# hanishkvc/prgs-sdr-kspecanal

Measured on AMD Instinct MI355X. Metric: windowed FFTs/sec, fftSize=4096, 50% overlap, hanning (zeroSpan hot path incl. Max/Min/Avg/Cur + waterfall), higher is better.
Workload: dtype f32

## Files before the change

prgs-sdr-kspecanal_amd/build.py:

```python
import os
import shutil
import subprocess
import sys

HERE = os.path.dirname(os.path.abspath(__file__))
SRC = os.path.join(HERE, "csrc", "ksa_api.hip")
OUT = os.path.join(HERE, "libksa.so")
FLAGS = ["--offload-arch=gfx950", "-O3", "-std=c++17", "-fno-slp-vectorize", "-Wno-unused-value",
         "-shared", "-fPIC"]


def sources():
    d = os.path.join(HERE, "csrc")
    return [os.path.join(d, f) for f in sorted(os.listdir(d))] + [os.path.join(HERE, "..", "include", "ksa.h")]


def is_stale():
    if not os.path.exists(OUT):
        return True
    t = os.path.getmtime(OUT)
    return any(os.path.getmtime(s) > t for s in sources())


def build(force=False, verbose=False):
    if not force and not is_stale():
        return OUT
    hipcc = shutil.which("hipcc") or "/opt/rocm/bin/hipcc"
    cmd = [hipcc] + FLAGS + ["-o", OUT + ".tmp", SRC]
    if verbose:
        print(" ".join(cmd))
    r = subprocess.run(cmd, capture_output=True, text=True)
    if r.returncode != 0:
        raise RuntimeError("hipcc failed:\n" + r.stdout + r.stderr)
    os.replace(OUT + ".tmp", OUT)
    return OUT


if __name__ == "__main__":
    print(build(force="--force" in sys.argv, verbose=True))
```

prgs-sdr-kspecanal_amd/csrc/ksa_api.hip:

```cpp
#include <hip/hip_runtime.h>

#include <algorithm>
#include <climits>
#include <cmath>
#include <cstdarg>
#include <cstdio>
#include <cstdlib>
#include <cstring>
#include <mutex>
#include <string>
#include <type_traits>
#include <vector>

#include "../../include/ksa.h"
#include "ksa_dif16.hpp"
#include "ksa_kernels.hpp"
#include "ksa_kernels32.hpp"
#include "ksa_kernels64.hpp"
#include "ksa_kernels_pair.hpp"
#include "ksa_kernels_mr.hpp"
#include "ksa_pfb.hpp"
#include "ksa_tables.hpp"

namespace {
// ... 55 lines not shown
  hipStream_t stream = nullptr;
  int num_cu = 0;
  int* d_starts = nullptr;
  int* d_start_last = nullptr;
  float* d_window = nullptr;
  float* d_window32 = nullptr;
  float2* d_tw_mid = nullptr;
  float2* d_tw_last = nullptr;
  float* d_adj = nullptr;
  float* d_scan_adj = nullptr;
  void* d_iq_stage = nullptr;
  float* d_frames = nullptr;
  float* d_part = nullptr;
  float* d_xchg = nullptr;
  float* d_partial = nullptr;
  float* d_state = nullptr;
  float* d_hm = nullptr;
  float* d_scan_state = nullptr;
  float* d_scan_hm = nullptr;
  float* d_scan_avg_rows = nullptr;
  float* d_levels = nullptr;
  int* d_highs = nullptr;
  float* d_parts = nullptr;
  int levels_cap = 0;
  float* d_gather = nullptr;
  size_t gather_cap = 0;
  void* d_scan_stage = nullptr;
  size_t scan_stage_cap = 0;
  float* d_scan_rows = nullptr;
  int scan_rows = 0;
  int scan_rows_passes = 0;
  float* d_scan_halo = nullptr;
  float* d_scan_send = nullptr;
  size_t scan_halo_cap = 0, scan_send_cap = 0;
  hipEvent_t ev_ready = nullptr, ev_copied = nullptr, ev_stream = nullptr;
  hipStream_t copy_stream = nullptr;
  void* d_slot[2] = {nullptr, nullptr};
  size_t slot_cap[2] = {0, 0};
  hipEvent_t ev_slot_copied[2] = {nullptr, nullptr}, ev_slot_read[2] = {nullptr, nullptr}, ev_copy_start = nullptr;
  float* d_host_rows = nullptr;
  size_t host_rows_cap = 0;
  int plan_frames = 0;
  int sub_n = 0;
  float2* d_dif_tw = nullptr;
  float2* d_dif_z = nullptr;
  float* d_dif_y = nullptr;
// ... 93 lines not shown
    return f(int_c<ksa::CUMU_AVG>{});
  }
  if (p.cumu == ksa::CUMU_AVG) return f(int_c<ksa::CUMU_AVG>{});
  if (p.cumu == ksa::CUMU_MAX) return f(int_c<ksa::CUMU_MAX>{});
  return f(int_c<ksa::CUMU_MIN>{});
}
constexpr bool fold_avg_or_psd(int cm) { return cm == ksa::CUMU_AVG || cm == ksa::CUMU_PSD; }

struct KernelFit {
  int vgprs = 0, blocks_per_cu = 1;
};
template <class K>
int configure_kernel(K kfn, int threads, int lds_bytes, KernelFit* fit, int lds_attr = -1) {
  HIP_OK(hipFuncSetAttribute(reinterpret_cast<const void*>(kfn), hipFuncAttributeMaxDynamicSharedMemorySize, lds_attr < 0 ? lds_bytes : lds_attr));
  hipFuncAttributes attr;
  HIP_OK(hipFuncGetAttributes(&attr, reinterpret_cast<const void*>(kfn)));
  int occ = 0;
  HIP_OK(hipOccupancyMaxActiveBlocksPerMultiprocessor(&occ, kfn, threads, lds_bytes));
  fit->vgprs = attr.numRegs;
  fit->blocks_per_cu = std::max(1, occ);
  return 0;
}

template <class K>
int launch_split(ksa_engine* e, K kfn, const SpecParams& p, int n, int threads, int lds_bytes, bool may_split, int grid_cap) {
  const int capacity = e->num_cu * e->blocks_per_cu;
  SpecParams q = p;
  const int plan = plan_of(e, p);
  if (e->d_parts && may_split && !exp_env("KSA_NO_SPLIT") && p.nwin > 1 && plan * 2 <= capacity) {
    q.parts = std::min(p.nwin, capacity / plan);
    q.part_out = e->d_parts;
  }
  int grid = std::max(1, std::min(q.nframes * std::max(1, q.parts), capacity));
  grid = std::max(1, std::min(grid, grid_cap));
  hipLaunchKernelGGL(kfn, dim3(grid), dim3(threads), lds_bytes, e->stream, q);
  if (q.parts > 1) {
    hipLaunchKernelGGL(ksa::combine_parts_kernel, dim3((n / 4 + 63) / 64, q.nframes), dim3(64), 0, e->stream, q, n);
    if (q.hm_w > 0)
      hipLaunchKernelGGL(ksa::rowmax_batch, dim3((q.hm_w + 255) / 256, q.nframes), dim3(256), 0, e->stream, q, n);
  }
  HIP_OK(hipGetLastError());
  return 0;
}

template <int N, int FMT, int RM, int CM>
int launch_pair_c(ksa_engine* e, const SpecParams& p, bool configure_only) {
  using PP = ksa::PlanPair<N>;
  auto kfn = ksa::spectrum_pair_kernel<N, FMT, RM, CM>;
  if (configure_only) {
    KernelFit fit;
    if (configure_kernel(kfn, ksa::Plan<N>::T, PP::LDS_BYTES, &fit)) return 1;
    if (FMT == ksa::FMT_C64 && fold_avg_or_psd(CM)) {
      e->pair_bpc = fit.blocks_per_cu;
      e->pair_vgprs = fit.vgprs;
      e->pair_lds = PP::LDS_BYTES;
    }
    return 0;
  }
  const int npairs = (p.nframes + 1) / 2;
  const int grid = std::max(1, std::min(npairs, e->num_cu * e->pair_bpc));
  hipLaunchKernelGGL(kfn, dim3(grid), dim3(ksa::Plan<N>::T), PP::LDS_BYTES, e->stream, p);
  HIP_OK(hipGetLastError());
  return 0;
}

template <int N, int FMT, int RM>
int launch_pair(ksa_engine* e, const SpecParams& p, bool cfg_only) {
  return with_fold(e, p, cfg_only, [&](auto cm) { return launch_pair_c<N, FMT, RM, decltype(cm)::value>(e, p, cfg_only); });
}

template <int N, int FMT, int RM, int CM>
int launch_spec_c(ksa_engine* e, const SpecParams& p, bool configure_only) {
  using P = ksa::Plan<N>;
  auto kfn = ksa::spectrum_kernel<N, FMT, RM, CM>;
  static const int lds_pad = exp_env("KSA_LDS_PAD_KB") ? atoi(exp_env("KSA_LDS_PAD_KB")) * 1024 : 0;
  const int lds_bytes = ksa::Tune<N>::LDS_BYTES + lds_pad;
  if (configure_only) {
    KernelFit fit;
    if (configure_kernel(kfn, P::T, lds_bytes, &fit)) return 1;
    if (FMT == ksa::FMT_C64) {
      e->threads = P::T;
      e->lds_bytes = ksa::Tune<N>::LDS_BYTES;
      e->vgprs = fit.vgprs;
      e->blocks_per_cu = fit.blocks_per_cu;
    }
    return 0;
  }
  return launch_split(e, kfn, p, N, P::T, lds_bytes, N >= 1024, INT_MAX);
}

template <int N, int FMT, int RM>
int launch_spec_t(ksa_engine* e, const SpecParams& p, bool configure_only) {
#ifdef KSA_EXPERIMENTS
  constexpr bool pair_size = ksa::Plan<N>::S == 1 && ksa::Plan<N>::T <= 256 && ksa::Plan<N>::M >= 2;
#else
  constexpr bool pair_size = N == 1024;
#endif
  if constexpr (pair_size) {
    if (e->pair_ok) {
      if (configure_only) {
        if (RM != 0 && launch_pair<N, FMT, 0>(e, p, true)) return 1;
        if (RM != 4 && launch_pair<N, FMT, 4>(e, p, true)) return 1;
        if (RM != 8 && launch_pair<N, FMT, 8>(e, p, true)) return 1;
        if (launch_pair<N, FMT, RM>(e, p, true)) return 1;
      } else if (plan_of(e, p) >= 2 * e->num_cu * e->pair_bpc) return launch_pair<N, FMT, RM>(e, p, false);
    }
  }
  if constexpr (ksa::Tune<N>::fold_const(RM)) {
    return with_fold(e, p, configure_only, [&](auto cm) { return launch_spec_c<N, FMT, RM, decltype(cm)::value>(e, p, configure_only); });
  } else {
    if (fold_psd(e)) return launch_spec_c<N, FMT, RM, ksa::CUMU_PSD>(e, p, configure_only);
// ... 26 lines not shown
    return 0;
  }
  const char* g = exp_env("KSA_GRID");
  return launch_split(e, kfn, p, N, P::T, P::LDS_BYTES, true, g ? atoi(g) : INT_MAX);
}

template <int N, int FMT>
int launch_spec32(ksa_engine* e, const SpecParams& p, bool cfg_only) {
  return with_fold(e, p, cfg_only, [&](auto cm) { return launch_spec32_c<N, FMT, decltype(cm)::value>(e, p, cfg_only); });
}

template <int CM, bool W1>
int launch_spec64_c(ksa_engine* e, const SpecParams& p, bool configure_only) {
  auto kfn = ksa::spectrum64_kernel<ksa::FMT_C64, CM, W1>;
  if (configure_only) {
    KernelFit fit;
    if (configure_kernel(kfn, ksa::Plan64::T, ksa::Plan64::LDS_BYTES, &fit)) return 1;
    if (fold_avg_or_psd(CM)) {
      e->k64_bpc = fit.blocks_per_cu;
      e->k64_vgprs = fit.vgprs;
    }
    return 0;
  }
  const int grid = std::max(1, std::min(p.nframes, e->num_cu * e->k64_bpc));
  hipLaunchKernelGGL(kfn, dim3(grid), dim3(ksa::Plan64::T), ksa::Plan64::LDS_BYTES, e->stream, p);
  HIP_OK(hipGetLastError());
  return 0;
}

int launch_spec64(ksa_engine* e, const SpecParams& p, bool cfg_only) {
  const bool w1 = e->win_ones && !exp_env("KSA_NO_W1");
  return with_fold(e, p, cfg_only, [&](auto cm) {
    constexpr int CM = decltype(cm)::value;
    return w1 ? launch_spec64_c<CM, true>(e, p, cfg_only) : launch_spec64_c<CM, false>(e, p, cfg_only);
  });
}

template <int FMT>
int launch_spec_n(ksa_engine* e, const SpecParams& p, bool cfg_only) {
  const int rm = p.nwin > 1 ? e->reuse_m : 0;
  if (e->plan32) return e->sub_n == 8192 ? launch_spec32<8192, FMT>(e, p, cfg_only) : launch_spec32<16384, FMT>(e, p, cfg_only);
  return with_size(e->sub_n, [&](auto size) {
    constexpr int N = decltype(size)::value;
    if constexpr (N == 64 && FMT == ksa::FMT_C64) {
      if (e->k64_ok) {
        if (cfg_only) { if (launch_spec64(e, p, true)) return 1; }
        else if (!exp_env("KSA_NO_K64")) return launch_spec64(e, p, false);
      }
// ... 151 lines not shown
          return dispatch(R, Radices{}, [&](auto radix) {
            constexpr int RX = decltype(radix)::value;
            if constexpr (RX == 16)
              hipLaunchKernelGGL(ksa::dif16_kernel<FMT>, dim3(n1 / 512, nwin, cf), dim3(256), 0, e->stream, a);
            else
              hipLaunchKernelGGL((ksa::dif_wide_kernel<FMT, RX>), dim3(n1 / 256, nwin, cf), dim3(256), 0, e->stream, a);
            return 0;
          });
        })) return 1;
    SpecParams b{};
    b.iq = e->d_dif_z;
    b.frame_stride = (long long)nwin * n1;
    b.frame_len = nwin * n1;
    b.nframes = cf * R;
    b.nwin = nwin;
    b.starts = e->d_starts_b;
    b.window = e->d_ones;
    b.tw_mid = p.tw_mid;
    b.tw_last = p.tw_last;
    b.scale = p.scale;
    b.cumu = p.cumu;
    b.out_mode = ksa::OUT_LINEAR;
    b.out = e->d_dif_y;
    e->plan_frames = chunk_frames * R;
    if (launch_spec_n<ksa::FMT_C64>(e, b, false)) return 1;
    ksa::DifFinishParams c{};
    c.y = e->d_dif_y;
    c.n = n;
    c.n1 = n1;
    c.radix = R;
    c.frame0 = f0;
    c.out_mode = p.out_mode;
    c.gain = p.gain;
    c.min_amp = p.min_amp;
    c.out = p.out;
    c.hm_w = p.hm_w;
    c.adj = p.adj;
    c.hm_rows = p.hm_rows;
    c.hm_ring = p.hm_ring;
    c.hm_index0 = p.hm_index0;
    c.hm_first = p.hm_first;
    dispatch(R, Radices{}, [&](auto radix) {
      hipLaunchKernelGGL(ksa::dif16_finish_kernel<decltype(radix)::value>, dim3(n1 / (1024 / R), cf), dim3(256), 0, e->stream, c);
      return 0;
    });
  }
// ... 28 lines not shown
  p.starts = raw ? e->d_start_last : e->d_starts;
#if defined(KSA32_TAPS_X4) && !KSA32_TAPS_X4
  p.window = e->d_window;
#else
  p.window = (e->plan32 && e->path == 0) ? e->d_window32 : e->d_window;
#endif
  p.tw_mid = e->d_tw_mid;
  p.tw_last = e->d_tw_last;
  p.scale = (float)c.mag_scale;
  p.cumu = (raw || fold || c.cumu_mode == KSA_CUMU_AVG || c.cumu_mode == KSA_CUMU_PSD) ? ksa::CUMU_AVG : c.cumu_mode == KSA_CUMU_MAX ? ksa::CUMU_MAX : ksa::CUMU_MIN;
  p.out_mode = out_mode;
  p.gain = c.gain;
  p.min_amp = c.min_amp;
  p.u8_offset = c.u8_offset;
  p.u8_inv_scale = 1.0f / c.u8_scale;
  p.out = out;
  p.hm_w = with_hm ? c.hm_width : 0;
  p.adj = with_hm ? e->d_adj : nullptr;
  p.hm_rows = with_hm ? hm_rows : nullptr;
  p.hm_ring = with_hm ? e->d_hm : nullptr;
  p.hm_index0 = (e->hm_index + f.batch_first) % KSA_HM_ROWS;
  p.hm_first = std::max(0, f.batch_frames - KSA_HM_ROWS - f.batch_first);
  e->plan_frames = f.batch_frames;
#ifdef KSA_STAMPS
  static unsigned long long* dbg = nullptr;
  const size_t dbg_n = 4096 * 16 * 12;
  if (!dbg) hipMalloc(reinterpret_cast<void**>(&dbg), dbg_n * 8);
  hipMemsetAsync(dbg, 0, dbg_n * 8, e->stream);
  p.dbg = dbg;
#endif
  ksa::u64x2* const clk = (e->prof && e->d_clk) ? reinterpret_cast<ksa::u64x2*>(e->d_clk) + (size_t)(e->clk_launches++ % ksa::CLK_SLOTS) * 2 * ksa::CLK_KEYS : nullptr;
  if (clk) hipLaunchKernelGGL(ksa::clock_stamp_kernel, dim3(ksa::CLK_WGS), dim3(64), 0, e->stream, clk, 0);
  hipEvent_t ea, eb;
  if (prof_begin(e, &ea, &eb)) return 1;
  if (fold && launch_pfb(e, *fold)) return 1;
  int rc;
  if (e->path == 2) rc = run_dif16(e, p, f.fmt, f.batch_first, f.batch_frames);
  else if (e->path == 6) rc = with_fmt(f.fmt, [&](auto fmt) { return launch_mr<decltype(fmt)::value>(e, p, false); });
  else rc = with_fmt(f.fmt, [&](auto fmt) { return launch_spec_n<decltype(fmt)::value>(e, p, false); });
  e->plan_frames = 0;
  if (rc) return rc;
#ifdef KSA_STAMPS
  if (const char* path = exp_env("KSA_STAMPS_FILE")) {
    hipStreamSynchronize(e->stream);
    std::vector<unsigned long long> h(dbg_n);
    hipMemcpy(h.data(), dbg, dbg_n * 8, hipMemcpyDeviceToHost);
    double sum[12] = {0};
    long long waves = 0;
    for (size_t w = 0; w < dbg_n / 12; ++w) {
      if (!h[w * 12 + 0] && !h[w * 12 + 7]) continue;
      ++waves;
      for (int i = 0; i < 12; ++i) sum[i] += (double)h[w * 12 + i];
    }
    if (FILE* fp = fopen(path, "a")) {
      fprintf(fp, "waves %lld nframes %d nwin %d :", waves, f.nframes, p.nwin);
      for (int i = 0; i < 12; ++i) fprintf(fp, " %.0f", waves ? sum[i] / waves : 0.0);
      fprintf(fp, "\n");
      fclose(fp);
    }
  }
#endif
  if (prof_end(e, ea, eb)) return 1;
  if (clk) hipLaunchKernelGGL(ksa::clock_stamp_kernel, dim3(ksa::CLK_WGS), dim3(64), 0, e->stream, clk, 1);
  return 0;
}

int run_spectrum(ksa_engine* e, Frames f, int out_mode, float* out, bool with_hm, float* hm_rows) {
  if (f.batch_frames < 1) f.batch_frames = f.nframes;
  if (!fold_time(e)) return run_transform(e, f, out_mode, out, with_hm, hm_rows, nullptr);
  const ksa_config& c = e->cfg;
  if (check_frames(e, f, out, hm_rows)) return 1;
  const size_t n = (size_t)c.fft_size;
  for (int f0 = 0; f0 < f.nframes; f0 += e->pfb_chunk) {
    const int nf = std::min(e->pfb_chunk, f.nframes - f0);
    const Frames fold{static_cast<const unsigned char*>(f.iq) + (size_t)f0 * (size_t)f.stride * sample_bytes(f.fmt), f.fmt, f.stride, nf};
    const Frames folded{e->d_pfb_y, KSA_FMT_C64, (long long)e->pfb_sub * c.fft_size, nf, f.batch_first + f0, f.batch_frames};
    if (run_transform(e, folded, out_mode, out + (size_t)f0 * n, with_hm, hm_rows ? hm_rows + (size_t)f0 * c.hm_width : nullptr, &fold)) return 1;
  }
  return 0;
}

int run_accumulate(ksa_engine* e, const float* db, int nframes, long long first_index, long long total) {
  const int n = e->cfg.fft_size;
  ksa::AccParams a{};
  a.db = db;
  a.n = n;
// ... 219 lines not shown
    if (const char* mb = exp_env("KSA_FS_SCRATCH_MB")) {
      const long v = atol(mb);
      if (v >= 1 && v <= (256l << 10)) budget = (size_t)v << 20;
    }
    e->dif_chunk = (int)std::min<size_t>(std::max<size_t>(1, budget / per_frame), (size_t)c.max_frames);
    e->dif_chunk = std::min(e->dif_chunk, 4095);
    if ((he = hipMalloc(reinterpret_cast<void**>(&e->d_dif_z), per_frame * e->dif_chunk)) != hipSuccess)
      return fail("hipMalloc(%zu) for the first-stage scratch: %s", per_frame * e->dif_chunk, hipGetErrorString(he));
    if ((he = hipMalloc(reinterpret_cast<void**>(&e->d_dif_y), (size_t)e->dif_chunk * n * 4)) != hipSuccess)
      return fail("hipMalloc for the second-stage output: %s", hipGetErrorString(he));
  }
  e->max_chunks = (int)std::max<size_t>(1, std::min<size_t>(128, (64u << 20) / (3 * nn * 4)));
#define ALLOC(ptr, bytes)                                                        \
  if ((he = hipMalloc(reinterpret_cast<void**>(&(ptr)), (bytes))) != hipSuccess) \
    return fail("hipMalloc(%zu) for %s: %s", (size_t)(bytes), #ptr, hipGetErrorString(he));
  ALLOC(e->d_iq_stage, (size_t)c.full_size * 8);
  ALLOC(e->d_frames, (size_t)c.max_frames * nn * 4);
  ALLOC(e->d_part, (size_t)e->max_chunks * 3 * nn * 4);
  ALLOC(e->d_xchg, (4 * nn + (size_t)KSA_HM_ROWS * c.hm_width) * 4);
  e->d_partial = e->d_xchg;
  if (c.hm_width) e->d_hm = e->d_xchg + 4 * nn;
  ALLOC(e->d_state, 4 * nn * 4);
  if (e->path != 6) ALLOC(e->d_parts, (size_t)e->num_cu * e->blocks_per_cu * (size_t)e->sub_n * 4);
  if (c.scan_total_entries) {
    ALLOC(e->d_scan_state, (size_t)4 * c.scan_total_entries * 4);
    ALLOC(e->d_scan_hm, (size_t)KSA_HM_ROWS * c.scan_hm_width * 4);
  }
#undef ALLOC
  return 0;
}

}

extern "C" {

int ksa_abi_version(void) { return KSA_ABI_VERSION; }
const char* ksa_last_error(void) { return g_err.c_str(); }

int ksa_create(const ksa_config* cfg, ksa_engine** out) {
  if (!cfg || !out) return fail("null argument");
  *out = nullptr;
  if (validate_config(cfg)) return 1;
  int ndev = 0;
  HIP_OK(hipGetDeviceCount(&ndev));
  if (cfg->device < 0 || cfg->device >= ndev) return fail("device %d not present (%d visible)", cfg->device, ndev);
  DeviceGuard dev_guard;
// ... 18 lines not shown
  if (upload_tables(e, cfg, w)) return bail(1);
  if (configure_kernels(e, w.num_windows)) return bail(1);
  if (alloc_scratch(e, w.num_windows)) return bail(1);
  if (ksa_reset_state(e)) return bail(1);
  if (cfg->scan_total_entries && scan_reset(e)) return bail(1);
  if (hipStreamSynchronize(e->stream) != hipSuccess) return bail(fail("initial sync failed"));
  *out = e;
  return 0;
}

void ksa_destroy(ksa_engine* e) {
  if (!e) return;
  DeviceGuard dev_guard;
  hipSetDevice(e->cfg.device);
  hipDeviceSynchronize();
  for (auto& pr : e->prof_events) { hipEventDestroy(pr.first); hipEventDestroy(pr.second); }
  for (hipEvent_t ev : {e->ev_ready, e->ev_copied, e->ev_stream, e->ev_copy_start, e->ev_slot_copied[0], e->ev_slot_copied[1],
                        e->ev_slot_read[0], e->ev_slot_read[1]})
    if (ev) hipEventDestroy(ev);
  if (e->copy_stream) hipStreamDestroy(e->copy_stream);
  void* ptrs[] = {e->d_slot[0], e->d_slot[1], e->d_host_rows, e->d_clk, e->d_gather, e->d_scan_stage, e->d_scan_rows, e->d_scan_halo, e->d_scan_send,
                  e->d_starts, e->d_start_last, e->d_window, e->d_window32, e->d_tw_mid, e->d_tw_last, e->d_adj, e->d_scan_adj,
                  e->d_iq_stage, e->d_frames, e->d_part, e->d_xchg, e->d_state, e->d_scan_state, e->d_scan_hm,
                  e->d_levels, e->d_parts, e->d_highs, e->d_scan_avg_rows, e->d_dif_tw, e->d_dif_z, e->d_dif_y, e->d_ones, e->d_starts_b,
                  e->d_pfb_starts, e->d_pfb_taps, e->d_pfb_y};
  for (void* p : ptrs) if (p) hipFree(p);
  delete e;
}

int ksa_set_stream(ksa_engine* e, void* hip_stream) {
  if (!e) return fail("null engine");
  hipStream_t ns = reinterpret_cast<hipStream_t>(hip_stream);
  if (ns == e->stream) return 0;
  DeviceGuard dev_guard;
  HIP_OK(hipSetDevice(e->cfg.device));
  if (!e->ev_stream) HIP_OK(hipEventCreateWithFlags(&e->ev_stream, hipEventDisableTiming));
  HIP_OK(hipEventRecord(e->ev_stream, e->stream));
  HIP_OK(hipStreamWaitEvent(ns, e->ev_stream, 0));
  e->stream = ns;
  return 0;
}

int ksa_synchronize(ksa_engine* e) {
  if (!e) return fail("null engine");
  DeviceGuard dev_guard;
  HIP_OK(hipSetDevice(e->cfg.device));
  HIP_OK(hipStreamSynchronize(e->stream));
// ... 864 lines not shown
```

prgs-sdr-kspecanal_amd/csrc/ksa_kernels.hpp:

```cpp
#pragma once
#include <hip/hip_runtime.h>
#include <stdint.h>
#include <type_traits>
#include "ksa_fft.hpp"

namespace ksa {

enum { CUMU_AVG = 1, CUMU_MAX = 2, CUMU_MIN = 3 };
enum { CUMU_PSD = 4 };
enum { OUT_LINEAR = 0, OUT_DB = 1, OUT_DB_CLIP = 2 };
enum { FMT_C64 = 0, FMT_U8 = 1, FMT_S8 = 2, FMT_S16 = 3 };
constexpr int HM_ROWS = 128;

struct SpecParams {
  const void* iq;
  long long frame_stride;
  int frame_len;
  int nframes;
  int nwin;
  const int* starts;
  const float* window;
  const float2* tw_mid;
  const float2* tw_last;
  float scale;
  int cumu;
  int out_mode;
  float gain, min_amp;
  float u8_offset, u8_inv_scale;
  float* out;
  int hm_w;
  const float* adj;
  float* hm_rows;
  float* hm_ring;
  int hm_index0;
  int hm_first;
  int parts;
  float* part_out;
  unsigned long long* dbg;
};

constexpr int CLK_WGS = 2048;
constexpr int CLK_KEYS = 4096;
constexpr int CLK_SLOTS = 16;
typedef unsigned long long u64x2 __attribute__((ext_vector_type(2)));
__global__ __launch_bounds__(64) void clock_stamp_kernel(u64x2* out, int which) {
  unsigned long long c, r;
  asm volatile("s_memtime %0\n\ts_memrealtime %1\n\ts_waitcnt lgkmcnt(0)" : "=s"(c), "=s"(r)::"memory");
  const unsigned xcc = __builtin_amdgcn_s_getreg(20 | (0 << 6) | ((4 - 1) << 11));
  const unsigned hw = __builtin_amdgcn_s_getreg(4 | (8 << 6) | ((8 - 1) << 11));
  if (threadIdx.x == 0) {
    u64x2 v;
    v.x = c;
    v.y = r;
    out[(size_t)which * CLK_KEYS + (((xcc & 15u) << 8) | (hw & 255u))] = v;
  }
}

__device__ __forceinline__ float db_of(float lin, float gain) { return fmaf(__builtin_amdgcn_logf(lin), 3.01029995663981195f, -gain); }

__device__ __forceinline__ float nan_max(float a, float b) { return __builtin_isunordered(a, b) ? __builtin_nanf("") : fmaxf(a, b); }
__device__ __forceinline__ float nan_min(float a, float b) { return __builtin_isunordered(a, b) ? __builtin_nanf("") : fminf(a, b); }
// ... 203 lines not shown
template <> struct RawOf<FMT_S8> { typedef unsigned int type; };
template <int FMT>
__device__ __forceinline__ float tap_scale(const SpecParams& p) { return FMT == FMT_U8 ? p.u8_inv_scale : fmt_fixed_scale(FMT); }
template <int FMT>
__device__ __forceinline__ float2 unpack_signed(unsigned b) {
  static_assert(FMT == FMT_S8 || FMT == FMT_S16, "signed fixed-point formats only");
  if constexpr (FMT == FMT_S8) return make_float2((float)(int)(signed char)(b & 0xff), (float)(int)(signed char)((b >> 8) & 0xff));
  else return make_float2((float)(int)(short)(b & 0xffff), (float)((int)b >> 16));
}

#ifdef KSA_STAMPS
#define KSA_STAMP(i)                                                                        \
  do {                                                                                      \
    __builtin_amdgcn_sched_barrier(0);                                                      \
    unsigned long long _t;                                                                  \
    asm volatile("s_memtime %0\n\ts_waitcnt lgkmcnt(0)" : "=s"(_t)::"memory");              \
    __builtin_amdgcn_sched_barrier(0);                                                      \
    seg[i] += _t - t_last;                                                                  \
    t_last = _t;                                                                            \
  } while (0)
#else
#define KSA_STAMP(i) do {} while (0)
#endif

#ifdef KSA_ABL_NOLDS
#define KSA_SYNC() do {} while (0)
#define KSA_LDS_ST(dst, val) do {} while (0)
#define KSA_LDS_LD(dst, src) do {} while (0)
#else
#ifdef KSA_LDS_BARRIER
#define KSA_SYNC() asm volatile("s_waitcnt lgkmcnt(0)\n\ts_barrier" ::: "memory")
#else
#define KSA_SYNC() __syncthreads()
#endif
#define KSA_LDS_ST(dst, val) (dst) = (val)
#ifndef KSA_LDS_ATOMIC_LD
#define KSA_LDS_ATOMIC_LD 1
#endif
__device__ __forceinline__ float2 lds_ld64(const float2* p) {
#if KSA_LDS_ATOMIC_LD
  const unsigned long long v = __atomic_load_n(reinterpret_cast<const unsigned long long*>(p), __ATOMIC_RELAXED);
  return make_float2(__uint_as_float((unsigned)v), __uint_as_float((unsigned)(v >> 32)));
#else
  return *p;
#endif
}
// ... 138 lines not shown
      else if constexpr (FMT == FMT_S16) raw[(q + ROT) & 15] = __builtin_amdgcn_raw_buffer_load_b32(rsrc, voff, L * q * SB, 0);
      else raw[(q + ROT) & 15] = __builtin_amdgcn_raw_buffer_load_b16(rsrc, voff, L * q * SB, 0);
#endif
    }
  };
  auto shift_raw = [&]() {
#pragma unroll
    for (int q = 0; q + RM < 16; ++q) raw[q] = raw[q + RM];
  };

#ifdef KSA_STAMPS
  unsigned long long seg[12] = {0, 0, 0, 0, 0, 0, 0, 0, 0, 0, 0, 0};
  unsigned long long t_last;
  asm volatile("s_memtime %0\n\ts_waitcnt lgkmcnt(0)" : "=s"(t_last)::"memory");
#endif
#ifndef KSA_PF
#define KSA_PF 1
#endif
  constexpr bool PF = KSA_PF && RM > 0 && N >= 2048;
#ifndef KSA_PP
#define KSA_PP 1
#endif
  constexpr bool PP = KSA_PP && PF && RM == 8 && N == 4096;
  for (int vf = blockIdx.x; vf < p.nframes * NP; vf += gridDim.x) {
    const int frame = vf / NP, part = vf - frame * NP;
    const int k_lo = (int)((long long)p.nwin * part / NP), k_hi = (int)((long long)p.nwin * (part + 1) / NP);
    const int rounds = (k_hi - k_lo + S - 1) / S;
    float acc[16];
    const float init = p.cumu == CUMU_MIN ? __builtin_inff() : 0.0f;
#pragma unroll
    for (int i = 0; i < 16; ++i) acc[i] = init;

    if constexpr (PP) {
      for (int rd0 = 0; rd0 < rounds; rd0 += 2) {
        {
          const int rd = rd0;
          constexpr int PAR = 0;
#include "ksa_window_body.inc"
        }
        if (rd0 + 1 < rounds) {
          const int rd = rd0 + 1;
          constexpr int PAR = 1;
#include "ksa_window_body.inc"
        }
      }
    } else {
      for (int rd = 0; rd < rounds; ++rd) {
        constexpr int PAR = 0;
#include "ksa_window_body.inc"
      }
    }

    float* const red = reinterpret_cast<float*>(lds);
    __syncthreads();
    KSA_STAMP(9);
#pragma unroll
    for (int i = 0; i < 16; ++i) red[slot * RedStride<N, S>::value + l + L * perm<16>(i)] = acc[i];
    __syncthreads();
    KSA_STAMP(10);
#ifdef KSA_ABL_NOFIN
    if (red[tid] == 123.456f) p.out[tid] = red[tid];
#else
    if (NP == 1) {
      finish_frame<N, T, S, CM>(p, red, frame, tid);
    } else {
      float4* const dst = reinterpret_cast<float4*>(p.part_out + (long long)vf * N);
      const float4* red4 = reinterpret_cast<const float4*>(red);
      for (int q = tid; q < N / 4; q += T) {
        float4 r = red4[q];
        if constexpr (S > 1) {
          for (int s2 = 1; s2 < S; ++s2) {
            const float4 x = red4[s2 * (RedStride<N, S>::value / 4) + q];
            if (CM == CUMU_PSD || p.cumu == CUMU_AVG) { r.x += x.x; r.y += x.y; r.z += x.z; r.w += x.w; }
            else if (p.cumu == CUMU_MAX) { r.x = nan_max(r.x, x.x); r.y = nan_max(r.y, x.y); r.z = nan_max(r.z, x.z); r.w = nan_max(r.w, x.w); }
            else { r.x = nan_min(r.x, x.x); r.y = nan_min(r.y, x.y); r.z = nan_min(r.z, x.z); r.w = nan_min(r.w, x.w); }
          }
        }
        dst[q] = r;
      }
    }
#endif
    KSA_STAMP(8);
  }
#ifdef KSA_STAMPS
  if (p.dbg && (tid & 63) == 0) {
    for (int i = 0; i < 12; ++i) p.dbg[((long long)blockIdx.x * (T / 64) + tid / 64) * 12 + i] = seg[i];
  }
#endif
}

__global__ void combine_parts_kernel(const SpecParams p, int n) {
  const int q = blockIdx.x * blockDim.x + threadIdx.x;
  if (q * 4 >= n) return;
  const int frame = blockIdx.y;
  const float4* src = reinterpret_cast<const float4*>(p.part_out + (long long)frame * p.parts * n) + q;
  float4 r = src[0];
  for (int part = 1; part < p.parts; ++part) {
    const float4 x = src[(long long)part * (n / 4)];
    if (p.cumu == CUMU_AVG) { r.x += x.x; r.y += x.y; r.z += x.z; r.w += x.w; }
    else if (p.cumu == CUMU_MAX) { r.x = nan_max(r.x, x.x); r.y = nan_max(r.y, x.y); r.z = nan_max(r.z, x.z); r.w = nan_max(r.w, x.w); }
    else { r.x = nan_min(r.x, x.x); r.y = nan_min(r.y, x.y); r.z = nan_min(r.z, x.z); r.w = nan_min(r.w, x.w); }
  }
  float o[4] = {r.x, r.y, r.z, r.w};
#pragma unroll
  for (int u = 0; u < 4; ++u) {
    float lin = p.cumu == CUMU_AVG ? o[u] : __builtin_amdgcn_sqrtf(o[u]);
// ... 450 lines not shown
```

prgs-sdr-kspecanal_amd/csrc/ksa_kernels32.hpp:

```cpp
#pragma once
#include <hip/hip_runtime.h>
#include <stdint.h>
#include <type_traits>

#include "ksa_kernels.hpp"

namespace ksa {

template <int N>
struct Plan32 {
  static_assert(N == 8192 || N == 16384, "32-point plan: N = 8192 or 16384");
  static constexpr int L = N / 32, T = L;
  static constexpr int R1 = N == 16384 ? 32 : 16;
  static constexpr int B1 = 32 / R1;
  static constexpr int P2 = 32 * R1;
  static constexpr int NPAD = N + N / 32;
  static constexpr int MID_ROWS = R1 == 32 ? 31 : 15;
  static constexpr int MID = MID_ROWS * 32;
  static constexpr int LDS_BYTES = (NPAD + MID) * 8;
  static constexpr int WPS = 2;
};

__host__ __device__ constexpr int pad32(int i) { return i + (i >> 5); }

// ... 105 lines not shown
      else if constexpr (FMT == FMT_S16) raw[q] = __builtin_amdgcn_raw_buffer_load_b32(rsrc, voff, L * q * SB, 0);
      else raw[q] = __builtin_amdgcn_raw_buffer_load_b16(rsrc, voff, L * q * SB, 0);
#endif
    }
  };
  auto k_lo_of = [&](int vf) { return (int)((long long)p.nwin * (vf % NP) / NP); };
  auto k_hi_of = [&](int vf) { return (int)((long long)p.nwin * (vf % NP + 1) / NP); };

#define PREFETCH_NEXT()                                      \
  do {                                                       \
    if constexpr (KSA32_PREFETCH) {                          \
      __builtin_amdgcn_sched_barrier(0);                     \
      issue_loads(vf, k + 1 < k_hi ? k + 1 : k);             \
      if constexpr (KSA32_PREFETCH == 2) load_taps();        \
      __builtin_amdgcn_sched_barrier(0);                     \
    }                                                        \
  } while (0)

#ifdef KSA_STAMPS
  unsigned long long seg[12] = {0, 0, 0, 0, 0, 0, 0, 0, 0, 0, 0, 0};
  unsigned long long t_last;
  asm volatile("s_memtime %0\n\ts_waitcnt lgkmcnt(0)" : "=s"(t_last)::"memory");
#endif
  for (int vf = blockIdx.x; vf < total; vf += gridDim.x) {
    const int frame = vf / NP;
    const int k_lo = k_lo_of(vf), k_hi = k_hi_of(vf);
    float acc[32];
    const float init = p.cumu == CUMU_MIN ? __builtin_inff() : 0.0f;
#pragma unroll
    for (int i = 0; i < 32; ++i) acc[i] = init;
    if constexpr (KSA32_PREFETCH) issue_loads(vf, k_lo);
    if constexpr (KSA32_PREFETCH == 2) load_taps();

    for (int k = k_lo; k < k_hi; ++k) {
      if constexpr (!KSA32_PREFETCH) issue_loads(vf, k);
      if constexpr (!KSA32_WIN_REGS && KSA32_PREFETCH != 2) load_taps();
      float2 v[32];
#pragma unroll
      for (int q = 0; q < 32; ++q) {
        if constexpr (FMT == FMT_C64) {
          const unsigned xr = raw[q].x, xi = raw[q].y;
          v[q] = make_float2(__uint_as_float(xr) * win[q], __uint_as_float(xi) * win[q]);
        } else if constexpr (FMT == FMT_S8 || FMT == FMT_S16) {
          const float2 x = unpack_signed<FMT>(raw[q]);
          v[q] = make_float2(x.x * win[q], x.y * win[q]);
        } else {
          const unsigned short x = raw[q];
// ... 84 lines not shown
          for (int i = 0; i < 16; ++i) acc[b * 16 + i] = nan_max_nonneg(acc[b * 16 + i], fmaf(u[i].x, u[i].x, u[i].y * u[i].y));
        } else {
#pragma unroll
          for (int i = 0; i < 16; ++i) acc[b * 16 + i] = nan_min(acc[b * 16 + i], fmaf(u[i].x, u[i].x, u[i].y * u[i].y));
        }
      }
      KSA_STAMP(6);
    }

    float* const red = reinterpret_cast<float*>(lds);
    __syncthreads();
#pragma unroll
    for (int i = 0; i < 32; ++i) red[l + L * ((i >> 4) + 2 * perm<16>(i & 15))] = acc[i];
    __syncthreads();
    if (NP == 1) {
      finish_frame<N, T, 1, CM>(p, red, frame, l);
    } else {
      float4* const dst = reinterpret_cast<float4*>(p.part_out + (long long)vf * N);
      const float4* red4 = reinterpret_cast<const float4*>(red);
      for (int q = l; q < N / 4; q += T) dst[q] = red4[q];
    }
    KSA_STAMP(8);
  }
#ifdef KSA_STAMPS
  if (p.dbg && (l & 63) == 0) {
    for (int i = 0; i < 12; ++i) p.dbg[((long long)blockIdx.x * (T / 64) + l / 64) * 12 + i] = seg[i];
  }
#endif
}

#undef PREFETCH_NEXT
#undef K32_ST
#undef K32_LD

}
```

prgs-sdr-kspecanal_amd/csrc/ksa_kernels64.hpp:

```cpp
#pragma once
#include <hip/hip_runtime.h>
#include <stdint.h>

#include "ksa_kernels.hpp"

namespace ksa {

struct Plan64 {
  static constexpr int N = 64, T = 64, S = 16, L = 4;
  static constexpr int XS = 68;
  static constexpr int LDS_BYTES = S * XS * 8 + N * 4;
};

template <int FMT, int CM, bool W1>
__global__ __launch_bounds__(64, 4) void spectrum64_kernel(const SpecParams p) {
  static_assert(FMT == FMT_C64, "adjacent-sample loads: complex64 input (16-byte loads of two samples)");
  using P = Plan64;
  constexpr int N = P::N, T = P::T, S = P::S;
  constexpr int SB = 8;
  extern __shared__ __attribute__((aligned(16))) float2 lds[];
  float* const taps_lds = reinterpret_cast<float*>(lds + S * P::XS);
  const int tid = threadIdx.x, slot = tid >> 2, l = tid & 3;
  float2* const my = lds + slot * P::XS;

  if constexpr (!W1) {
    const int n = tid, lp = (n & 7) >> 1, c = n & 1, j = n >> 3;
    taps_lds[lp * 16 + 2 * j + c] = p.window[n];
  }
  float2 twb[7];
#pragma unroll
  for (int k1 = 1; k1 < 8; ++k1) twb[k1 - 1] = p.tw_mid[(2 * l) * 8 + k1];
  __syncthreads();

  const int nm1 = p.nwin - 1;
  const int rounds = (p.nwin + S - 1) / S;
#ifdef KSA_STAMPS
  unsigned long long seg[12] = {0, 0, 0, 0, 0, 0, 0, 0, 0, 0, 0, 0};
  unsigned long long t_last;
  asm volatile("s_memtime %0\n\ts_waitcnt lgkmcnt(0)" : "=s"(t_last)::"memory");
#endif
  typedef unsigned int u32x4 __attribute__((ext_vector_type(4)));
  for (int frame = blockIdx.x; frame < p.nframes; frame += gridDim.x) {
    float acc[16];
    const float init = p.cumu == CUMU_MIN ? __builtin_inff() : 0.0f;
#pragma unroll
    for (int i = 0; i < 16; ++i) acc[i] = init;
    const char* fbase = reinterpret_cast<const char*>(p.iq) + (long long)frame * p.frame_stride * SB;
    const auto rsrc = __builtin_amdgcn_make_buffer_rsrc(const_cast<char*>(fbase), 0, p.frame_len * SB, 0x00020000);

    for (int rd = 0; rd < rounds; ++rd) {
      const int k = rd * S + slot;
      const bool active = k < p.nwin;
      float2 v[16];
      if (active) {
        const int voff = (p.starts[k] + 2 * l) * SB;
        u32x4 piece[8];
#pragma unroll
        for (int j = 0; j < 8; ++j) piece[j] = __builtin_amdgcn_raw_buffer_load_b128(rsrc, voff, 8 * j * SB, 0);
        KSA_STAMP(11);
#pragma unroll
        for (int j = 0; j < 8; ++j) {
          const float2 w2 = W1 ? make_float2(1.0f, 1.0f) : reinterpret_cast<const float2*>(taps_lds)[l * 8 + j];
          const unsigned a = piece[j].x, b = piece[j].y, c = piece[j].z, d = piece[j].w;
          if constexpr (W1) {
            v[j] = make_float2(__uint_as_float(a), __uint_as_float(b));
// ... 44 lines not shown
        KSA_STAMP(6);
        const int cm = CM == 0 ? p.cumu : CM;
        if constexpr (CM == CUMU_PSD) {
#pragma unroll
          for (int i = 0; i < 16; ++i) acc[i] = fmaf(u[i].x, u[i].x, fmaf(u[i].y, u[i].y, acc[i]));
        } else if (cm == CUMU_AVG) {
          const int e = k == 0 ? nm1 : nm1 - k + 1;
          const float wgt = ldexpf(1.0f, -e);
#pragma unroll
          for (int i = 0; i < 16; ++i)
            acc[i] = fmaf(wgt, __builtin_amdgcn_sqrtf(fmaf(u[i].x, u[i].x, u[i].y * u[i].y)), acc[i]);
        } else if (cm == CUMU_MAX) {
#pragma unroll
          for (int i = 0; i < 16; ++i) acc[i] = nan_max_nonneg(acc[i], fmaf(u[i].x, u[i].x, u[i].y * u[i].y));
        } else {
#pragma unroll
          for (int i = 0; i < 16; ++i) acc[i] = nan_min(acc[i], fmaf(u[i].x, u[i].x, u[i].y * u[i].y));
        }
      }
      KSA_STAMP(7);
    }
    float* const red = reinterpret_cast<float*>(lds);
    __syncthreads();
#pragma unroll
    for (int c = 0; c < 2; ++c)
#pragma unroll
      for (int Pp = 0; Pp < 8; ++Pp) red[slot * RedStride<N, S>::value + (2 * l + c) + 8 * perm<8>(Pp)] = acc[c * 8 + Pp];
    __syncthreads();
    KSA_STAMP(10);
    finish_frame<N, T, S, CM>(p, red, frame, tid);
    KSA_STAMP(8);
  }
#ifdef KSA_STAMPS
  if (p.dbg && tid == 0)
    for (int i = 0; i < 12; ++i) p.dbg[(long long)blockIdx.x * 12 + i] = seg[i];
#endif
}

}
```

prgs-sdr-kspecanal_amd/csrc/ksa_kernels_pair.hpp:

```cpp
#pragma once
#include <hip/hip_runtime.h>
#include <stdint.h>
#include <type_traits>

#include "ksa_fft_pair.hpp"
#include "ksa_kernels.hpp"

namespace ksa {

template <int N>
struct PlanPair {
  using P = Plan<N>;
  static_assert(P::S == 1 && P::T <= 256 && P::M >= 2, "pair kernel: one transform per workgroup, N = 1024 .. 4096");
  static constexpr bool XLAYOUT = KSA_XLAYOUT && N == 1024;
  static constexpr int ST1 = 260, K2 = 4, SH2 = 6;
  static constexpr int NPAD = XLAYOUT ? 1084 : P::N_PLUS_PAD16;
  static constexpr int LDS_BYTES = NPAD * 16 + P::MID * 8;
  static_assert(4 * N * 4 <= NPAD * 16, "output planes must fit the exchange buffer");
};

template <int N, int FMT, int RM, int CM>
__global__ __launch_bounds__(Plan<N>::T, 2) void spectrum_pair_kernel(const SpecParams p) {
  using P = Plan<N>;
  using PP = PlanPair<N>;
// ... 32 lines not shown
    const char* ba = reinterpret_cast<const char*>(p.iq) + (long long)fa * p.frame_stride * SB;
    const char* bb = reinterpret_cast<const char*>(p.iq) + (long long)fb * p.frame_stride * SB;
    const auto rsa = __builtin_amdgcn_make_buffer_rsrc(const_cast<char*>(ba), 0, p.frame_len * SB, 0x00020000);
    const auto rsb = __builtin_amdgcn_make_buffer_rsrc(const_cast<char*>(bb), 0, p.frame_len * SB, 0x00020000);
    const int start = RM > 0 ? start0 + k * (RM * L) : p.starts[k];
    const int voff = (start + l) * SB;
#pragma unroll
    for (int q = 0; q < 16; ++q) {
      if (q < q0) continue;
      if constexpr (FMT == FMT_C64) {
        ra[q] = __builtin_amdgcn_raw_buffer_load_b64(rsa, voff, L * q * SB, 0);
        rb[q] = __builtin_amdgcn_raw_buffer_load_b64(rsb, voff, L * q * SB, 0);
      } else if constexpr (FMT == FMT_S16) {
        ra[q] = __builtin_amdgcn_raw_buffer_load_b32(rsa, voff, L * q * SB, 0);
        rb[q] = __builtin_amdgcn_raw_buffer_load_b32(rsb, voff, L * q * SB, 0);
      } else {
        ra[q] = __builtin_amdgcn_raw_buffer_load_b16(rsa, voff, L * q * SB, 0);
        rb[q] = __builtin_amdgcn_raw_buffer_load_b16(rsb, voff, L * q * SB, 0);
      }
    }
  };

  const int npairs = (p.nframes + 1) / 2;
  for (int pf = blockIdx.x; pf < npairs; pf += gridDim.x) {
    const int fa = 2 * pf;
    const bool has_b = fa + 1 < p.nframes;
    const int fb = has_b ? fa + 1 : fa;
    v2f acc[16];
    const float init = p.cumu == CUMU_MIN ? __builtin_inff() : 0.0f;
#pragma unroll
    for (int i = 0; i < 16; ++i) acc[i] = splat(init);

    for (int k = 0; k < p.nwin; ++k) {
      issue_loads(fa, fb, k, (RM > 0 && k > 0) ? 16 - RM : 0);
      cx2 v[16];
#pragma unroll
      for (int q = 0; q < 16; ++q) {
        cx2 e;
        if constexpr (FMT == FMT_C64) {
          const unsigned ar = ra[q].x, ai = ra[q].y, br = rb[q].x, bi = rb[q].y;
          e.x.x = __uint_as_float(ar) * win[q]; e.x.y = __uint_as_float(br) * win[q];
          e.y.x = __uint_as_float(ai) * win[q]; e.y.y = __uint_as_float(bi) * win[q];
        } else if constexpr (FMT == FMT_S8 || FMT == FMT_S16) {
          const float2 xa = unpack_signed<FMT>(ra[q]), xb = unpack_signed<FMT>(rb[q]);
          e.x.x = xa.x * win[q]; e.x.y = xb.x * win[q];
          e.y.x = xa.y * win[q]; e.y.y = xb.y * win[q];
        } else {
// ... 68 lines not shown
        const v2f w = splat(ldexpf(1.0f, -e));
#pragma unroll
        for (int i = 0; i < 16; ++i) {
          const v2f m2 = fma2(v[i].x, v[i].x, v[i].y * v[i].y);
          acc[i] = fma2(w, v2f{__builtin_amdgcn_sqrtf(m2.x), __builtin_amdgcn_sqrtf(m2.y)}, acc[i]);
        }
      } else if (cm == CUMU_MAX) {
#pragma unroll
        for (int i = 0; i < 16; ++i) {
          const v2f m2 = fma2(v[i].x, v[i].x, v[i].y * v[i].y);
          acc[i] = v2f{nan_max_nonneg(acc[i].x, m2.x), nan_max_nonneg(acc[i].y, m2.y)};
        }
      } else {
#pragma unroll
        for (int i = 0; i < 16; ++i) {
          const v2f m2 = fma2(v[i].x, v[i].x, v[i].y * v[i].y);
          acc[i] = v2f{nan_min(acc[i].x, m2.x), nan_min(acc[i].y, m2.y)};
        }
      }
    }

    float* const red = reinterpret_cast<float*>(lds2);
    __syncthreads();
#pragma unroll
    for (int i = 0; i < 16; ++i) {
      red[l + L * perm<16>(i)] = acc[i].x;
      red[2 * N + l + L * perm<16>(i)] = acc[i].y;
    }
    __syncthreads();
    finish_frame<N, T, 1, CM>(p, red, fa, l);
    if (has_b) finish_frame<N, T, 1, CM>(p, red + 2 * N, fb, l);
  }
}

}
```

Baseline: 178.7 million.

## Replace static grid-stride frame walk with atomic ticket-based dynamic scheduling

The spectrum, pair and 64-point kernels now take their next frame (or run of frames) from a global atomic ticket counter instead of striding by gridDim. The aim is to balance load across workgroups when per-unit cost is skewed, cutting tail imbalance. The counter is reset with a memset before each launch, and the ticket is broadcast through LDS with an extra barrier. The change also adds skew-timing instrumentation behind a compile flag and a parallel experiments build.

```diff
diff --git a/prgs-sdr-kspecanal_amd/build.py b/prgs-sdr-kspecanal_amd/build.py
--- a/prgs-sdr-kspecanal_amd/build.py
+++ b/prgs-sdr-kspecanal_amd/build.py
@@ -6,6 +6,7 @@
 HERE = os.path.dirname(os.path.abspath(__file__))
 SRC = os.path.join(HERE, "csrc", "ksa_api.hip")
 OUT = os.path.join(HERE, "libksa.so")
+OUT_EXP = os.path.join(HERE, "libksa_exp.so")
 FLAGS = ["--offload-arch=gfx950", "-O3", "-std=c++17", "-fno-slp-vectorize", "-Wno-unused-value",
          "-shared", "-fPIC"]
 
@@ -15,24 +16,32 @@
     return [os.path.join(d, f) for f in sorted(os.listdir(d))] + [os.path.join(HERE, "..", "include", "ksa.h")]
 
 
-def is_stale():
-    if not os.path.exists(OUT):
+def is_stale(out=OUT):
+    if not os.path.exists(out):
         return True
-    t = os.path.getmtime(OUT)
+    t = os.path.getmtime(out)
     return any(os.path.getmtime(s) > t for s in sources())
 
 
 def build(force=False, verbose=False):
-    if not force and not is_stale():
-        return OUT
     hipcc = shutil.which("hipcc") or "/opt/rocm/bin/hipcc"
-    cmd = [hipcc] + FLAGS + ["-o", OUT + ".tmp", SRC]
-    if verbose:
-        print(" ".join(cmd))
-    r = subprocess.run(cmd, capture_output=True, text=True)
-    if r.returncode != 0:
-        raise RuntimeError("hipcc failed:\n" + r.stdout + r.stderr)
-    os.replace(OUT + ".tmp", OUT)
+    jobs = []
+    for out, extra in ((OUT, []), (OUT_EXP, ["-DKSA_EXPERIMENTS"])):
+        if not force and not is_stale(out):
+            continue
+        cmd = [hipcc] + FLAGS + extra + ["-o", out + ".tmp", SRC]
+        if verbose:
+            print(" ".join(cmd))
+        jobs.append((out, subprocess.Popen(cmd, stdout=subprocess.PIPE, stderr=subprocess.STDOUT, text=True)))
+    failed = []
+    for out, proc in jobs:
+        log = proc.communicate()[0]
+        if proc.returncode != 0:
+            failed.append(log)
+        else:
+            os.replace(out + ".tmp", out)
+    if failed:
+        raise RuntimeError("hipcc failed:\n" + "\n".join(failed))
     return OUT
 
 
diff --git a/prgs-sdr-kspecanal_amd/csrc/ksa_api.hip b/prgs-sdr-kspecanal_amd/csrc/ksa_api.hip
--- a/prgs-sdr-kspecanal_amd/csrc/ksa_api.hip
+++ b/prgs-sdr-kspecanal_amd/csrc/ksa_api.hip
@@ -101,6 +101,7 @@
   float* d_levels = nullptr;
   int* d_highs = nullptr;
   float* d_parts = nullptr;
+  unsigned* d_tickets = nullptr;
   int levels_cap = 0;
   float* d_gather = nullptr;
   size_t gather_cap = 0;
@@ -240,8 +241,9 @@
   return 0;
 }
 
+constexpr long long TICKET_MIN_POINTS = 5 * 4096;
 template <class K>
-int launch_split(ksa_engine* e, K kfn, const SpecParams& p, int n, int threads, int lds_bytes, bool may_split, int grid_cap) {
+int launch_split(ksa_engine* e, K kfn, const SpecParams& p, int n, int threads, int lds_bytes, bool may_split, int grid_cap, bool tickets = false) {
   const int capacity = e->num_cu * e->blocks_per_cu;
   SpecParams q = p;
   const int plan = plan_of(e, p);
@@ -251,6 +253,10 @@
   }
   int grid = std::max(1, std::min(q.nframes * std::max(1, q.parts), capacity));
   grid = std::max(1, std::min(grid, grid_cap));
+  if (tickets && e->d_tickets && !exp_env("KSA_STATIC_WALK") && (long long)(p.nwin / std::max(1, q.parts)) * n >= TICKET_MIN_POINTS) {
+    HIP_OK(hipMemsetAsync(e->d_tickets, 0, sizeof(unsigned), e->stream));
+    q.tickets = e->d_tickets;
+  }
   hipLaunchKernelGGL(kfn, dim3(grid), dim3(threads), lds_bytes, e->stream, q);
   if (q.parts > 1) {
     hipLaunchKernelGGL(ksa::combine_parts_kernel, dim3((n / 4 + 63) / 64, q.nframes), dim3(64), 0, e->stream, q, n);
@@ -259,6 +265,19 @@
   }
   HIP_OK(hipGetLastError());
   return 0;
+}
+
+int ticket_runs(ksa_engine* e, SpecParams& q, int units, long long points, int cap) {
+  if (const char* g = exp_env("KSA_GRID")) cap = std::max(1, std::min(cap, atoi(g)));
+  const int run = (int)std::max<long long>(1, (TICKET_MIN_POINTS + points - 1) / std::max<long long>(1, points));
+  q.ticket_run = 1;
+  if (e->d_tickets && !exp_env("KSA_STATIC_WALK") && units >= 2ll * cap * run) {
+    if (hipMemsetAsync(e->d_tickets, 0, sizeof(unsigned), e->stream) != hipSuccess) return -1;
+    q.tickets = e->d_tickets;
+    q.ticket_run = run;
+    return cap;
+  }
+  return std::max(1, std::min(units, cap));
 }
 
 template <int N, int FMT, int RM, int CM>
@@ -276,8 +295,10 @@
     return 0;
   }
   const int npairs = (p.nframes + 1) / 2;
-  const int grid = std::max(1, std::min(npairs, e->num_cu * e->pair_bpc));
-  hipLaunchKernelGGL(kfn, dim3(grid), dim3(ksa::Plan<N>::T), PP::LDS_BYTES, e->stream, p);
+  SpecParams q = p;
+  const int grid = ticket_runs(e, q, npairs, 2ll * p.nwin * N, e->num_cu * e->pair_bpc);
+  if (grid < 0) return fail("hipMemsetAsync of the ticket counter failed");
+  hipLaunchKernelGGL(kfn, dim3(grid), dim3(ksa::Plan<N>::T), PP::LDS_BYTES, e->stream, q);
   HIP_OK(hipGetLastError());
   return 0;
 }
@@ -304,7 +325,8 @@
     }
     return 0;
   }
-  return launch_split(e, kfn, p, N, P::T, lds_bytes, N >= 1024, INT_MAX);
+  const char* g = exp_env("KSA_GRID");
+  return launch_split(e, kfn, p, N, P::T, lds_bytes, N >= 1024, g ? atoi(g) : INT_MAX, P::S == 1);
 }
 
 template <int N, int FMT, int RM>
@@ -377,8 +399,10 @@
     }
     return 0;
   }
-  const int grid = std::max(1, std::min(p.nframes, e->num_cu * e->k64_bpc));
-  hipLaunchKernelGGL(kfn, dim3(grid), dim3(ksa::Plan64::T), ksa::Plan64::LDS_BYTES, e->stream, p);
+  SpecParams q = p;
+  const int grid = ticket_runs(e, q, p.nframes, (long long)p.nwin * ksa::Plan64::N, e->num_cu * e->k64_bpc);
+  if (grid < 0) return fail("hipMemsetAsync of the ticket counter failed");
+  hipLaunchKernelGGL(kfn, dim3(grid), dim3(ksa::Plan64::T), ksa::Plan64::LDS_BYTES, e->stream, q);
   HIP_OK(hipGetLastError());
   return 0;
 }
@@ -576,6 +600,7 @@
     b.cumu = p.cumu;
     b.out_mode = ksa::OUT_LINEAR;
     b.out = e->d_dif_y;
+    b.dbg = p.dbg;
     e->plan_frames = chunk_frames * R;
     if (launch_spec_n<ksa::FMT_C64>(e, b, false)) return 1;
     ksa::DifFinishParams c{};
@@ -650,11 +675,11 @@
   p.hm_index0 = (e->hm_index + f.batch_first) % KSA_HM_ROWS;
   p.hm_first = std::max(0, f.batch_frames - KSA_HM_ROWS - f.batch_first);
   e->plan_frames = f.batch_frames;
-#ifdef KSA_STAMPS
+#ifdef KSA_SKEW
   static unsigned long long* dbg = nullptr;
-  const size_t dbg_n = 4096 * 16 * 12;
-  if (!dbg) hipMalloc(reinterpret_cast<void**>(&dbg), dbg_n * 8);
-  hipMemsetAsync(dbg, 0, dbg_n * 8, e->stream);
+  const size_t dbg_n = ksa::SKEW_SEG_WORDS, skew_n = (size_t)ksa::SKEW_WGS * 4;
+  if (!dbg) hipMalloc(reinterpret_cast<void**>(&dbg), (dbg_n + skew_n) * 8);
+  hipMemsetAsync(dbg, 0, (dbg_n + skew_n) * 8, e->stream);
   p.dbg = dbg;
 #endif
   ksa::u64x2* const clk = (e->prof && e->d_clk) ? reinterpret_cast<ksa::u64x2*>(e->d_clk) + (size_t)(e->clk_launches++ % ksa::CLK_SLOTS) * 2 * ksa::CLK_KEYS : nullptr;
@@ -690,6 +715,21 @@
 #endif
   if (prof_end(e, ea, eb)) return 1;
   if (clk) hipLaunchKernelGGL(ksa::clock_stamp_kernel, dim3(ksa::CLK_WGS), dim3(64), 0, e->stream, clk, 1);
+#ifdef KSA_SKEW
+  if (const char* path = getenv("KSA_SKEW_FILE")) {
+    static int skew_launch = 0;
+    hipStreamSynchronize(e->stream);
+    std::vector<unsigned long long> h(skew_n);
+    hipMemcpy(h.data(), dbg + dbg_n, skew_n * 8, hipMemcpyDeviceToHost);
+    if (FILE* fp = fopen(path, "a")) {
+      for (int w = 0; w < ksa::SKEW_WGS; ++w)
+        if (h[w * 4 + 1])
+          fprintf(fp, "launch %d %d %llu %llu %llu %llu\n", skew_launch, w, h[w * 4 + 3], h[w * 4 + 0], h[w * 4 + 1], h[w * 4 + 2]);
+      fclose(fp);
+    }
+    ++skew_launch;
+  }
+#endif
   return 0;
 }
 
@@ -955,6 +995,7 @@
   if (c.hm_width) e->d_hm = e->d_xchg + 4 * nn;
   ALLOC(e->d_state, 4 * nn * 4);
   if (e->path != 6) ALLOC(e->d_parts, (size_t)e->num_cu * e->blocks_per_cu * (size_t)e->sub_n * 4);
+  ALLOC(e->d_tickets, sizeof(unsigned));
   if (c.scan_total_entries) {
     ALLOC(e->d_scan_state, (size_t)4 * c.scan_total_entries * 4);
     ALLOC(e->d_scan_hm, (size_t)KSA_HM_ROWS * c.scan_hm_width * 4);
@@ -1019,7 +1060,7 @@
   void* ptrs[] = {e->d_slot[0], e->d_slot[1], e->d_host_rows, e->d_clk, e->d_gather, e->d_scan_stage, e->d_scan_rows, e->d_scan_halo, e->d_scan_send,
                   e->d_starts, e->d_start_last, e->d_window, e->d_window32, e->d_tw_mid, e->d_tw_last, e->d_adj, e->d_scan_adj,
                   e->d_iq_stage, e->d_frames, e->d_part, e->d_xchg, e->d_state, e->d_scan_state, e->d_scan_hm,
-                  e->d_levels, e->d_parts, e->d_highs, e->d_scan_avg_rows, e->d_dif_tw, e->d_dif_z, e->d_dif_y, e->d_ones, e->d_starts_b,
+                  e->d_levels, e->d_parts, e->d_tickets, e->d_highs, e->d_scan_avg_rows, e->d_dif_tw, e->d_dif_z, e->d_dif_y, e->d_ones, e->d_starts_b,
                   e->d_pfb_starts, e->d_pfb_taps, e->d_pfb_y};
   for (void* p : ptrs) if (p) hipFree(p);
   delete e;
diff --git a/prgs-sdr-kspecanal_amd/csrc/ksa_kernels.hpp b/prgs-sdr-kspecanal_amd/csrc/ksa_kernels.hpp
--- a/prgs-sdr-kspecanal_amd/csrc/ksa_kernels.hpp
+++ b/prgs-sdr-kspecanal_amd/csrc/ksa_kernels.hpp
@@ -37,6 +37,8 @@
   int parts;
   float* part_out;
   unsigned long long* dbg;
+  unsigned* tickets;
+  int ticket_run;
 };
 
 constexpr int CLK_WGS = 2048;
@@ -286,6 +288,38 @@
 #else
 #define KSA_STAMP(i) do {} while (0)
 #endif
+#if defined(KSA_STAMPS) && !defined(KSA_SKEW)
+#define KSA_SKEW 1
+#endif
+constexpr int SKEW_WGS = 4096;
+constexpr size_t SKEW_SEG_WORDS = (size_t)4096 * 16 * 12;
+#ifdef KSA_SKEW
+__device__ __forceinline__ void skew_store(unsigned long long* dbg, int word, unsigned long long v) {
+  if (dbg && threadIdx.x == 0 && blockIdx.x < SKEW_WGS) dbg[SKEW_SEG_WORDS + (size_t)blockIdx.x * 4 + word] = v;
+}
+#define KSA_SKEW_BEGIN() int skew_units = 0; skew_store(p.dbg, 0, wall_clock64())
+#define KSA_SKEW_UNIT() ++skew_units
+#define KSA_SKEW_END()                                                                                      \
+  do {                                                                                                      \
+    skew_store(p.dbg, 1, wall_clock64());                                                                   \
+    skew_store(p.dbg, 2, (unsigned long long)skew_units);                                                   \
+    skew_store(p.dbg, 3, __builtin_amdgcn_s_getreg(20 | (0 << 6) | ((4 - 1) << 11)));    \
+  } while (0)
+#else
+#define KSA_SKEW_BEGIN() do {} while (0)
+#define KSA_SKEW_UNIT() do {} while (0)
+#define KSA_SKEW_END() do {} while (0)
+#endif
+
+template <int T>
+__device__ __forceinline__ int ticket_next(unsigned ticket, unsigned* word) {
+  if constexpr (T > 64) {
+    if (threadIdx.x == 0) *word = ticket;
+    __syncthreads();
+    ticket = *word;
+  }
+  return (int)(gridDim.x + (unsigned)__builtin_amdgcn_readfirstlane((int)ticket));
+}
 
 #ifdef KSA_ABL_NOLDS
 #define KSA_SYNC() do {} while (0)
@@ -470,7 +504,13 @@
 #define KSA_PP 1
 #endif
   constexpr bool PP = KSA_PP && PF && RM == 8 && N == 4096;
-  for (int vf = blockIdx.x; vf < p.nframes * NP; vf += gridDim.x) {
+  constexpr bool TICKETS = S == 1;
+  static_assert(!TICKETS || NPAD > N, "the ticket word lies behind the output stage's two planes of N floats");
+  const int units = p.nframes * NP;
+  unsigned* const next_unit = reinterpret_cast<unsigned*>(lds + S * NPAD) - 1;
+  KSA_SKEW_BEGIN();
+  for (int vf = blockIdx.x; vf < units;) {
+    KSA_SKEW_UNIT();
     const int frame = vf / NP, part = vf - frame * NP;
     const int k_lo = (int)((long long)p.nwin * part / NP), k_hi = (int)((long long)p.nwin * (part + 1) / NP);
     const int rounds = (k_hi - k_lo + S - 1) / S;
@@ -502,6 +542,10 @@
     float* const red = reinterpret_cast<float*>(lds);
     __syncthreads();
     KSA_STAMP(9);
+    unsigned ticket = 0;
+    if constexpr (TICKETS) {
+      if (p.tickets && tid == 0) ticket = __hip_atomic_fetch_add(p.tickets, 1u, __ATOMIC_RELAXED, __HIP_MEMORY_SCOPE_AGENT);
+    }
 #pragma unroll
     for (int i = 0; i < 16; ++i) red[slot * RedStride<N, S>::value + l + L * perm<16>(i)] = acc[i];
     __syncthreads();
@@ -529,7 +573,10 @@
     }
 #endif
     KSA_STAMP(8);
-  }
+    if (TICKETS && p.tickets) vf = ticket_next<T>(ticket, next_unit);
+    else vf += gridDim.x;
+  }
+  KSA_SKEW_END();
 #ifdef KSA_STAMPS
   if (p.dbg && (tid & 63) == 0) {
     for (int i = 0; i < 12; ++i) p.dbg[((long long)blockIdx.x * (T / 64) + tid / 64) * 12 + i] = seg[i];
diff --git a/prgs-sdr-kspecanal_amd/csrc/ksa_kernels32.hpp b/prgs-sdr-kspecanal_amd/csrc/ksa_kernels32.hpp
--- a/prgs-sdr-kspecanal_amd/csrc/ksa_kernels32.hpp
+++ b/prgs-sdr-kspecanal_amd/csrc/ksa_kernels32.hpp
@@ -151,7 +151,9 @@
   unsigned long long t_last;
   asm volatile("s_memtime %0\n\ts_waitcnt lgkmcnt(0)" : "=s"(t_last)::"memory");
 #endif
+  KSA_SKEW_BEGIN();
   for (int vf = blockIdx.x; vf < total; vf += gridDim.x) {
+    KSA_SKEW_UNIT();
     const int frame = vf / NP;
     const int k_lo = k_lo_of(vf), k_hi = k_hi_of(vf);
     float acc[32];
@@ -282,6 +284,7 @@
     }
     KSA_STAMP(8);
   }
+  KSA_SKEW_END();
 #ifdef KSA_STAMPS
   if (p.dbg && (l & 63) == 0) {
     for (int i = 0; i < 12; ++i) p.dbg[((long long)blockIdx.x * (T / 64) + l / 64) * 12 + i] = seg[i];
diff --git a/prgs-sdr-kspecanal_amd/csrc/ksa_kernels64.hpp b/prgs-sdr-kspecanal_amd/csrc/ksa_kernels64.hpp
--- a/prgs-sdr-kspecanal_amd/csrc/ksa_kernels64.hpp
+++ b/prgs-sdr-kspecanal_amd/csrc/ksa_kernels64.hpp
@@ -40,7 +40,11 @@
   asm volatile("s_memtime %0\n\ts_waitcnt lgkmcnt(0)" : "=s"(t_last)::"memory");
 #endif
   typedef unsigned int u32x4 __attribute__((ext_vector_type(4)));
-  for (int frame = blockIdx.x; frame < p.nframes; frame += gridDim.x) {
+  const int run_len = p.tickets ? p.ticket_run : 1;
+  int run = blockIdx.x, frame = run * run_len, f_hi = min(frame + run_len, p.nframes);
+  KSA_SKEW_BEGIN();
+  while (frame < p.nframes) {
+    KSA_SKEW_UNIT();
     float acc[16];
     const float init = p.cumu == CUMU_MIN ? __builtin_inff() : 0.0f;
 #pragma unroll
@@ -131,6 +135,9 @@
     }
     float* const red = reinterpret_cast<float*>(lds);
     __syncthreads();
+    const bool run_ends = frame + 1 == f_hi;
+    unsigned ticket = 0;
+    if (p.tickets && run_ends && tid == 0) ticket = __hip_atomic_fetch_add(p.tickets, 1u, __ATOMIC_RELAXED, __HIP_MEMORY_SCOPE_AGENT);
 #pragma unroll
     for (int c = 0; c < 2; ++c)
 #pragma unroll
@@ -139,7 +146,14 @@
     KSA_STAMP(10);
     finish_frame<N, T, S, CM>(p, red, frame, tid);
     KSA_STAMP(8);
+    ++frame;
+    if (run_ends) {
+      run = p.tickets ? ticket_next<T>(ticket, nullptr) : run + (int)gridDim.x;
+      frame = run * run_len;
+      f_hi = min(frame + run_len, p.nframes);
+    }
   }
+  KSA_SKEW_END();
 #ifdef KSA_STAMPS
   if (p.dbg && tid == 0)
     for (int i = 0; i < 12; ++i) p.dbg[(long long)blockIdx.x * 12 + i] = seg[i];
diff --git a/prgs-sdr-kspecanal_amd/csrc/ksa_kernels_pair.hpp b/prgs-sdr-kspecanal_amd/csrc/ksa_kernels_pair.hpp
--- a/prgs-sdr-kspecanal_amd/csrc/ksa_kernels_pair.hpp
+++ b/prgs-sdr-kspecanal_amd/csrc/ksa_kernels_pair.hpp
@@ -78,7 +78,13 @@
   };
 
   const int npairs = (p.nframes + 1) / 2;
-  for (int pf = blockIdx.x; pf < npairs; pf += gridDim.x) {
+  static_assert(4 * N * 4 + 4 <= NPAD * 16, "the ticket word sits behind the output planes");
+  unsigned* const next_word = reinterpret_cast<unsigned*>(lds2 + NPAD) - 1;
+  const int run_len = p.tickets ? p.ticket_run : 1;
+  int run = blockIdx.x, pf = run * run_len, pf_hi = min(pf + run_len, npairs);
+  KSA_SKEW_BEGIN();
+  while (pf < npairs) {
+    KSA_SKEW_UNIT();
     const int fa = 2 * pf;
     const bool has_b = fa + 1 < p.nframes;
     const int fb = has_b ? fa + 1 : fa;
@@ -193,6 +199,9 @@
 
     float* const red = reinterpret_cast<float*>(lds2);
     __syncthreads();
+    const bool run_ends = pf + 1 == pf_hi;
+    unsigned ticket = 0;
+    if (p.tickets && run_ends && l == 0) ticket = __hip_atomic_fetch_add(p.tickets, 1u, __ATOMIC_RELAXED, __HIP_MEMORY_SCOPE_AGENT);
 #pragma unroll
     for (int i = 0; i < 16; ++i) {
       red[l + L * perm<16>(i)] = acc[i].x;
@@ -201,7 +210,14 @@
     __syncthreads();
     finish_frame<N, T, 1, CM>(p, red, fa, l);
     if (has_b) finish_frame<N, T, 1, CM>(p, red + 2 * N, fb, l);
+    ++pf;
+    if (run_ends) {
+      run = p.tickets ? ticket_next<T>(ticket, next_word) : run + (int)gridDim.x;
+      pf = run * run_len;
+      pf_hi = min(pf + run_len, npairs);
+    }
   }
+  KSA_SKEW_END();
 }
 
 }
```

Result: faster. 207.6 million (median of 6 runs) (+16.2%).
